# jiaw-z/DKT-Stereo

Measured on AMD Instinct MI355X. Metric: stereo pairs/sec at 736x1248 D=192, 32 iters (RAFT-Stereo test_mode forward), higher is better.
Workload: dtype f32 io/accumulate; convolution products = 3x fp16-split MFMA (22-bit operands); lookup / correlation exact fp32

## Files before the change

dkt_stereo_amd/csrc/resample_c8.hip:

```cpp
#include "dkt_common.h"

__device__ __forceinline__ unsigned rs_pack_h2(_Float16 a, _Float16 b) {
    union { _Float16 h[2]; unsigned u; } v;
    v.h[0] = a;
    v.h[1] = b;
    return v.u;
}

__device__ __forceinline__ void rs_store_c8(char *p, long plane, const float (&v)[8], float scale) {
    unsigned hw[4], lw[4];
#pragma unroll
    for (int d = 0; d < 4; ++d) {
        const float x0 = v[2 * d] * scale, x1 = v[2 * d + 1] * scale;
        const _Float16 a0 = (_Float16)x0, a1 = (_Float16)x1;
        hw[d] = rs_pack_h2(a0, a1);
        lw[d] = rs_pack_h2((_Float16)(x0 - (float)a0), (_Float16)(x1 - (float)a1));
    }
    *(uint4 *)p = make_uint4(hw[0], hw[1], hw[2], hw[3]);
    *(uint4 *)(p + plane) = make_uint4(lw[0], lw[1], lw[2], lw[3]);
}

__device__ __forceinline__ void pool2x_c8_body(const float *__restrict__ x, long x_bs, char *__restrict__ dst, long dst_bs,
                                               int C, int H, int W, int Ho, int Wo, int Wp, long plane, int ch0, float scale,
                                               int bx, int oy, int bz) {
    const int ox = bx * 128 + threadIdx.x;
    const int g = bz % ((C + 7) / 8), b = bz / ((C + 7) / 8);
    if (ox >= Wo) return;
    const float *xb = x + (long)b * x_bs;
    float v[8];
#pragma unroll
    for (int k = 0; k < 8; ++k) {
        const int c = g * 8 + k;
        const float *p = xb + (long)(c < C ? c : C - 1) * H * W;
        float t[9];
#pragma unroll
        for (int dy = 0; dy < 3; ++dy) {
            const int iy = 2 * oy - 1 + dy;
            const bool yok = iy >= 0 && iy < H;
#pragma unroll
            for (int dx = 0; dx < 3; ++dx) {
                const int ix = 2 * ox - 1 + dx;
                const bool ok = yok && ix >= 0 && ix < W;
                const float u = p[(long)(yok ? iy : 0) * W + (ix >= 0 && ix < W ? ix : 0)];
                t[dy * 3 + dx] = ok ? u : 0.0f;
            }
        }
        float s = 0.0f;
#pragma unroll
        for (int i = 0; i < 9; ++i) s = __fadd_rn(s, t[i]);
        v[k] = c < C ? __fdiv_rn(s, 9.0f) : 0.0f;
    }
    rs_store_c8(dst + (long)b * dst_bs + (long)((ch0 >> 3) + g) * 2 * plane + ((long)(oy + 1) * Wp + (ox + 1)) * 16, plane, v, scale);
}

__device__ __forceinline__ void interp_c8_body(const float *__restrict__ x, long x_bs, char *__restrict__ dst, long dst_bs,
                                               int C, int H, int W, int Ho, int Wo, float sy, float sx, int Wp, long plane,
                                               int ch0, float scale, int bx, int oy, int bz) {
    const int ox = bx * 128 + threadIdx.x;
    const int g = bz % ((C + 7) / 8), b = bz / ((C + 7) / 8);
    if (ox >= Wo) return;
    const float fy = __fmul_rn(sy, (float)oy);
    const int y0 = (int)fy;
    const int y1 = y0 + (y0 < H - 1 ? 1 : 0);
    const float ly1 = __fsub_rn(fy, (float)y0), ly0 = __fsub_rn(1.0f, ly1);
    const float fx = __fmul_rn(sx, (float)ox);
    const int x0 = (int)fx;
    const int x1 = x0 + (x0 < W - 1 ? 1 : 0);
    const float lx1 = __fsub_rn(fx, (float)x0), lx0 = __fsub_rn(1.0f, lx1);
    const float *xb = x + (long)b * x_bs;
    float a0[8], a1[8], b0[8], b1[8];
#pragma unroll
    for (int k = 0; k < 8; ++k) {
        const int c = g * 8 + k;
        const float *p = xb + (long)(c < C ? c : C - 1) * H * W;
        a0[k] = p[(long)y0 * W + x0]; a1[k] = p[(long)y0 * W + x1];
        b0[k] = p[(long)y1 * W + x0]; b1[k] = p[(long)y1 * W + x1];
    }
    float v[8];
#pragma unroll
    for (int k = 0; k < 8; ++k) {
        const float top = __fadd_rn(__fmul_rn(lx0, a0[k]), __fmul_rn(lx1, a1[k]));
        const float bot = __fadd_rn(__fmul_rn(lx0, b0[k]), __fmul_rn(lx1, b1[k]));
        v[k] = g * 8 + k < C ? __fadd_rn(__fmul_rn(ly0, top), __fmul_rn(ly1, bot)) : 0.0f;
    }
    rs_store_c8(dst + (long)b * dst_bs + (long)((ch0 >> 3) + g) * 2 * plane + ((long)(oy + 1) * Wp + (ox + 1)) * 16, plane, v, scale);
}

__global__ __launch_bounds__(128) void pool2x_c8_kernel(const float *__restrict__ x, long x_bs, char *__restrict__ dst, long dst_bs,
                                                        int C, int H, int W, int Ho, int Wo, int Wp, long plane, int ch0, float scale) {
    pool2x_c8_body(x, x_bs, dst, dst_bs, C, H, W, Ho, Wo, Wp, plane, ch0, scale, blockIdx.x, blockIdx.y, blockIdx.z);
}

__global__ __launch_bounds__(128) void interp_c8_kernel(const float *__restrict__ x, long x_bs, char *__restrict__ dst, long dst_bs,
                                                        int C, int H, int W, int Ho, int Wo, float sy, float sx, int Wp, long plane,
                                                        int ch0, float scale) {
    interp_c8_body(x, x_bs, dst, dst_bs, C, H, W, Ho, Wo, sy, sx, Wp, plane, ch0, scale, blockIdx.x, blockIdx.y, blockIdx.z);
}

struct RsJob {
    const float *x; long x_bs;
    char *dst; long dst_bs;
    int C, H, W, Ho, Wo, Wp; long plane; int ch0; float scale;
    float sy, sx;
    int kind;
    int nbx, nby;
};
struct RsPair { RsJob j[2]; };

__global__ __launch_bounds__(128) void resample_pair_c8_kernel(RsPair a, int nb0) {
    const bool second = (int)blockIdx.x >= nb0;
    const RsJob &j = a.j[second ? 1 : 0];
    int id = (int)blockIdx.x - (second ? nb0 : 0);
    const int bx = id % j.nbx; id /= j.nbx;
    const int oy = id % j.nby, bz = id / j.nby;
    if (j.kind == 0) pool2x_c8_body(j.x, j.x_bs, j.dst, j.dst_bs, j.C, j.H, j.W, j.Ho, j.Wo, j.Wp, j.plane, j.ch0, j.scale, bx, oy, bz);
    else interp_c8_body(j.x, j.x_bs, j.dst, j.dst_bs, j.C, j.H, j.W, j.Ho, j.Wo, j.sy, j.sx, j.Wp, j.plane, j.ch0, j.scale, bx, oy, bz);
}

static int rs_fill(RsJob &j, const dkt_resample_c8_job *d, long &blocks) {
    if (!d || !d->x || !d->dst) return DKT_E_NULL;
    if (d->B <= 0 || d->C <= 0 || d->H <= 0 || d->W <= 0 || (d->ch0 & 7) || !(d->scale > 0.0f)) return DKT_E_SHAPE;
    if (d->kind != 0 && d->kind != 1) return DKT_E_UNSUPPORTED;
    j.x = d->x; j.x_bs = d->x_bstride; j.dst = (char *)d->dst; j.dst_bs = d->dst_bstride_bytes;
    j.C = d->C; j.H = d->H; j.W = d->W; j.ch0 = d->ch0; j.scale = d->scale; j.kind = d->kind;
    if (d->kind == 0) {
        j.Ho = (d->H - 1) / 2 + 1; j.Wo = (d->W - 1) / 2 + 1;
        j.sy = j.sx = 0.0f;
    } else {
        if (d->Ho <= 0 || d->Wo <= 0) return DKT_E_SHAPE;
        j.Ho = d->Ho; j.Wo = d->Wo;
        j.sy = j.Ho > 1 ? (float)(d->H - 1) / (float)(j.Ho - 1) : 0.0f;
        j.sx = j.Wo > 1 ? (float)(d->W - 1) / (float)(j.Wo - 1) : 0.0f;
    }
    int Hp, Wp;
    dkt_act_c8_dims(j.Ho, j.Wo, &Hp, &Wp);
    j.Wp = Wp; j.plane = (long)Hp * Wp * 16;
    j.nbx = (j.Wo + 127) / 128; j.nby = j.Ho;
    blocks = (long)j.nbx * j.nby * d->B * ((d->C + 7) / 8);
    return DKT_OK;
}

extern "C" int dkt_resample_pair_c8(const dkt_resample_c8_job *job0, const dkt_resample_c8_job *job1, int device, void *stream) {
    RsPair a;
    long n0 = 0, n1 = 0;
    int rc = rs_fill(a.j[0], job0, n0);
    if (rc != DKT_OK) return rc;
    rc = rs_fill(a.j[1], job1, n1);
    if (rc != DKT_OK) return rc;
    if (n0 + n1 > 0x7fffffffL) return DKT_E_SHAPE;
    DKT_ENTER(device);
    hipLaunchKernelGGL(resample_pair_c8_kernel, dim3((unsigned)(n0 + n1)), dim3(128), 0, (hipStream_t)stream, a, (int)n0);
    return dkt_launch_status();
}

extern "C" int dkt_pool2x_c8(const float *x, long x_bstride, void *dst, long dst_bstride_bytes, int B, int C, int H, int W,
                             int ch0, float scale, int device, void *stream) {
    if (!x || !dst) return DKT_E_NULL;
    if (B <= 0 || C <= 0 || H <= 0 || W <= 0 || (ch0 & 7) || !(scale > 0.0f)) return DKT_E_SHAPE;
    const int Ho = (H - 1) / 2 + 1, Wo = (W - 1) / 2 + 1;
    int Hp, Wp;
    dkt_act_c8_dims(Ho, Wo, &Hp, &Wp);
    const long gz = (long)B * ((C + 7) / 8);
    if (gz > 65535 || Ho > 65535) return DKT_E_SHAPE;
    DKT_ENTER(device);
    hipLaunchKernelGGL(pool2x_c8_kernel, dim3((unsigned)((Wo + 127) / 128), (unsigned)Ho, (unsigned)gz), dim3(128), 0, (hipStream_t)stream,
                       x, x_bstride, (char *)dst, dst_bstride_bytes, C, H, W, Ho, Wo, Wp, (long)Hp * Wp * 16, ch0, scale);
    return dkt_launch_status();
}

extern "C" int dkt_interp_c8(const float *x, long x_bstride, void *dst, long dst_bstride_bytes, int B, int C, int H, int W,
                             int Ho, int Wo, int ch0, float scale, int device, void *stream) {
    if (!x || !dst) return DKT_E_NULL;
    if (B <= 0 || C <= 0 || H <= 0 || W <= 0 || Ho <= 0 || Wo <= 0 || (ch0 & 7) || !(scale > 0.0f)) return DKT_E_SHAPE;
    int Hp, Wp;
    dkt_act_c8_dims(Ho, Wo, &Hp, &Wp);
    const long gz = (long)B * ((C + 7) / 8);
    if (gz > 65535 || Ho > 65535) return DKT_E_SHAPE;
    const float sy = Ho > 1 ? (float)(H - 1) / (float)(Ho - 1) : 0.0f;
    const float sx = Wo > 1 ? (float)(W - 1) / (float)(Wo - 1) : 0.0f;
    DKT_ENTER(device);
    hipLaunchKernelGGL(interp_c8_kernel, dim3((unsigned)((Wo + 127) / 128), (unsigned)Ho, (unsigned)gz), dim3(128), 0, (hipStream_t)stream,
                       x, x_bstride, (char *)dst, dst_bstride_bytes, C, H, W, Ho, Wo, sy, sx, Wp, (long)Hp * Wp * 16, ch0, scale);
    return dkt_launch_status();
}
```

Before: 31.57.

## Stage resample input tiles in LDS with strip-based tiling for pool and interp

```diff
diff --git a/dkt_stereo_amd/csrc/resample_c8.hip b/dkt_stereo_amd/csrc/resample_c8.hip
--- a/dkt_stereo_amd/csrc/resample_c8.hip
+++ b/dkt_stereo_amd/csrc/resample_c8.hip
@@ -20,82 +20,10 @@
     *(uint4 *)(p + plane) = make_uint4(lw[0], lw[1], lw[2], lw[3]);
 }
 
-__device__ __forceinline__ void pool2x_c8_body(const float *__restrict__ x, long x_bs, char *__restrict__ dst, long dst_bs,
-                                               int C, int H, int W, int Ho, int Wo, int Wp, long plane, int ch0, float scale,
-                                               int bx, int oy, int bz) {
-    const int ox = bx * 128 + threadIdx.x;
-    const int g = bz % ((C + 7) / 8), b = bz / ((C + 7) / 8);
-    if (ox >= Wo) return;
-    const float *xb = x + (long)b * x_bs;
-    float v[8];
-#pragma unroll
-    for (int k = 0; k < 8; ++k) {
-        const int c = g * 8 + k;
-        const float *p = xb + (long)(c < C ? c : C - 1) * H * W;
-        float t[9];
-#pragma unroll
-        for (int dy = 0; dy < 3; ++dy) {
-            const int iy = 2 * oy - 1 + dy;
-            const bool yok = iy >= 0 && iy < H;
-#pragma unroll
-            for (int dx = 0; dx < 3; ++dx) {
-                const int ix = 2 * ox - 1 + dx;
-                const bool ok = yok && ix >= 0 && ix < W;
-                const float u = p[(long)(yok ? iy : 0) * W + (ix >= 0 && ix < W ? ix : 0)];
-                t[dy * 3 + dx] = ok ? u : 0.0f;
-            }
-        }
-        float s = 0.0f;
-#pragma unroll
-        for (int i = 0; i < 9; ++i) s = __fadd_rn(s, t[i]);
-        v[k] = c < C ? __fdiv_rn(s, 9.0f) : 0.0f;
-    }
-    rs_store_c8(dst + (long)b * dst_bs + (long)((ch0 >> 3) + g) * 2 * plane + ((long)(oy + 1) * Wp + (ox + 1)) * 16, plane, v, scale);
-}
-
-__device__ __forceinline__ void interp_c8_body(const float *__restrict__ x, long x_bs, char *__restrict__ dst, long dst_bs,
-                                               int C, int H, int W, int Ho, int Wo, float sy, float sx, int Wp, long plane,
-                                               int ch0, float scale, int bx, int oy, int bz) {
-    const int ox = bx * 128 + threadIdx.x;
-    const int g = bz % ((C + 7) / 8), b = bz / ((C + 7) / 8);
-    if (ox >= Wo) return;
-    const float fy = __fmul_rn(sy, (float)oy);
-    const int y0 = (int)fy;
-    const int y1 = y0 + (y0 < H - 1 ? 1 : 0);
-    const float ly1 = __fsub_rn(fy, (float)y0), ly0 = __fsub_rn(1.0f, ly1);
-    const float fx = __fmul_rn(sx, (float)ox);
-    const int x0 = (int)fx;
-    const int x1 = x0 + (x0 < W - 1 ? 1 : 0);
-    const float lx1 = __fsub_rn(fx, (float)x0), lx0 = __fsub_rn(1.0f, lx1);
-    const float *xb = x + (long)b * x_bs;
-    float a0[8], a1[8], b0[8], b1[8];
-#pragma unroll
-    for (int k = 0; k < 8; ++k) {
-        const int c = g * 8 + k;
-        const float *p = xb + (long)(c < C ? c : C - 1) * H * W;
-        a0[k] = p[(long)y0 * W + x0]; a1[k] = p[(long)y0 * W + x1];
-        b0[k] = p[(long)y1 * W + x0]; b1[k] = p[(long)y1 * W + x1];
-    }
-    float v[8];
-#pragma unroll
-    for (int k = 0; k < 8; ++k) {
-        const float top = __fadd_rn(__fmul_rn(lx0, a0[k]), __fmul_rn(lx1, a1[k]));
-        const float bot = __fadd_rn(__fmul_rn(lx0, b0[k]), __fmul_rn(lx1, b1[k]));
-        v[k] = g * 8 + k < C ? __fadd_rn(__fmul_rn(ly0, top), __fmul_rn(ly1, bot)) : 0.0f;
-    }
-    rs_store_c8(dst + (long)b * dst_bs + (long)((ch0 >> 3) + g) * 2 * plane + ((long)(oy + 1) * Wp + (ox + 1)) * 16, plane, v, scale);
-}
-
-__global__ __launch_bounds__(128) void pool2x_c8_kernel(const float *__restrict__ x, long x_bs, char *__restrict__ dst, long dst_bs,
-                                                        int C, int H, int W, int Ho, int Wo, int Wp, long plane, int ch0, float scale) {
-    pool2x_c8_body(x, x_bs, dst, dst_bs, C, H, W, Ho, Wo, Wp, plane, ch0, scale, blockIdx.x, blockIdx.y, blockIdx.z);
-}
-
-__global__ __launch_bounds__(128) void interp_c8_kernel(const float *__restrict__ x, long x_bs, char *__restrict__ dst, long dst_bs,
-                                                        int C, int H, int W, int Ho, int Wo, float sy, float sx, int Wp, long plane,
-                                                        int ch0, float scale) {
-    interp_c8_body(x, x_bs, dst, dst_bs, C, H, W, Ho, Wo, sy, sx, Wp, plane, ch0, scale, blockIdx.x, blockIdx.y, blockIdx.z);
-}
+#define RS_THREADS 256
+#define RS_LDS_FLOATS 6144
+#define RS_MAX_ROWS 8
+#define RS_MAX_ITEMS 768
 
 struct RsJob {
     const float *x; long x_bs;
@@ -104,17 +32,141 @@
     float sy, sx;
     int kind;
     int nbx, nby;
+    int R, XS, pitch;
 };
 struct RsPair { RsJob j[2]; };
 
-__global__ __launch_bounds__(128) void resample_pair_c8_kernel(RsPair a, int nb0) {
+#define RS_BATCH 6
+__device__ __forceinline__ void rs_stage(float *lds, const float *__restrict__ xb, int C, int H, int W, int g, int y_lo, int ns,
+                                         int cb, int pitch) {
+    const int Q = pitch >> 2, n = ns * 8 * Q;
+    for (int i0 = threadIdx.x; i0 < n; i0 += RS_BATCH * RS_THREADS) {
+        float4 v[RS_BATCH];
+        int at[RS_BATCH];
+#pragma unroll
+        for (int u = 0; u < RS_BATCH; ++u) {
+            const int i = i0 + u * RS_THREADS;
+            const int rk = i / Q, q = i - rk * Q;
+            const int c = g * 8 + (rk & 7), iy = y_lo + (rk >> 3), ix = cb + 4 * q;
+            at[u] = i < n ? rk * pitch + 4 * q : -1;
+            v[u] = make_float4(0.0f, 0.0f, 0.0f, 0.0f);
+            if (i < n && c < C && iy >= 0 && iy < H) {
+                const float *row = xb + ((long)c * H + iy) * W;
+                if (ix >= 0 && ix + 3 < W && (((uintptr_t)(row + ix)) & 15) == 0) {
+                    v[u] = *(const float4 *)(row + ix);
+                } else {
+                    if (ix >= 0 && ix < W) v[u].x = row[ix];
+                    if (ix + 1 >= 0 && ix + 1 < W) v[u].y = row[ix + 1];
+                    if (ix + 2 >= 0 && ix + 2 < W) v[u].z = row[ix + 2];
+                    if (ix + 3 >= 0 && ix + 3 < W) v[u].w = row[ix + 3];
+                }
+            }
+        }
+#pragma unroll
+        for (int u = 0; u < RS_BATCH; ++u)
+            if (at[u] >= 0) *(float4 *)(lds + at[u]) = v[u];
+    }
+}
+
+__device__ __forceinline__ void pool2x_c8_strip(float *lds, const RsJob &j, int seg, int strip, int bz) {
+    const int G = (j.C + 7) / 8, g = bz % G, b = bz / G;
+    const int oy0 = strip * j.R, nr = min(j.R, j.Ho - oy0);
+    const int ox0 = seg * j.XS, nx = min(j.XS, j.Wo - ox0);
+    const int pitch = j.pitch;
+    rs_stage(lds, j.x + (long)b * j.x_bs, j.C, j.H, j.W, g, 2 * oy0 - 1, 2 * nr + 1, 2 * ox0 - 4, pitch);
+    __syncthreads();
+    char *db = j.dst + (long)b * j.dst_bs + (long)((j.ch0 >> 3) + g) * 2 * j.plane;
+    for (int item = threadIdx.x; item < nr * nx; item += RS_THREADS) {
+        const int r = item / nx, lx = item - r * nx;
+        const float *tap = lds + (long)(2 * r) * 8 * pitch + 2 * lx + 3;
+        float v[8];
+#pragma unroll
+        for (int k = 0; k < 8; ++k) {
+            float t[9];
+#pragma unroll
+            for (int dy = 0; dy < 3; ++dy) {
+                const float *q = tap + (dy * 8 + k) * pitch;
+                const float2 m = *(const float2 *)(q + 1);
+                t[dy * 3] = q[0]; t[dy * 3 + 1] = m.x; t[dy * 3 + 2] = m.y;
+            }
+            float s = 0.0f;
+#pragma unroll
+            for (int i = 0; i < 9; ++i) s = __fadd_rn(s, t[i]);
+            v[k] = g * 8 + k < j.C ? __fdiv_rn(s, 9.0f) : 0.0f;
+        }
+        rs_store_c8(db + ((long)(oy0 + r + 1) * j.Wp + (ox0 + lx + 1)) * 16, j.plane, v, j.scale);
+    }
+}
+
+__device__ __forceinline__ void interp_c8_strip(float *lds, const RsJob &j, int seg, int strip, int bz) {
+    const int G = (j.C + 7) / 8, g = bz % G, b = bz / G;
+    const int H = j.H, W = j.W;
+    const int oy0 = strip * j.R, nr = min(j.R, j.Ho - oy0);
+    const int ox0 = seg * j.XS, nx = min(j.XS, j.Wo - ox0);
+    const int pitch = j.pitch;
+    const int ylo = (int)__fmul_rn(j.sy, (float)oy0);
+    const int ylast = (int)__fmul_rn(j.sy, (float)(oy0 + nr - 1));
+    const int ns = min(ylast + (ylast < H - 1 ? 1 : 0) - ylo + 1, RS_LDS_FLOATS / (8 * pitch));
+    const int cb = (int)__fmul_rn(j.sx, (float)ox0) & ~3;
+    rs_stage(lds, j.x + (long)b * j.x_bs, j.C, H, W, g, ylo, ns, cb, pitch);
+    __syncthreads();
+    char *db = j.dst + (long)b * j.dst_bs + (long)((j.ch0 >> 3) + g) * 2 * j.plane;
+    for (int item = threadIdx.x; item < nr * nx; item += RS_THREADS) {
+        const int r = item / nx, lx = item - r * nx;
+        const int oy = oy0 + r, ox = ox0 + lx;
+        const float fy = __fmul_rn(j.sy, (float)oy);
+        const int y0 = (int)fy;
+        const int y1 = y0 + (y0 < H - 1 ? 1 : 0);
+        const float ly1 = __fsub_rn(fy, (float)y0), ly0 = __fsub_rn(1.0f, ly1);
+        const float fx = __fmul_rn(j.sx, (float)ox);
+        const int x0 = (int)fx;
+        const int x1 = x0 + (x0 < W - 1 ? 1 : 0);
+        const float lx1 = __fsub_rn(fx, (float)x0), lx0 = __fsub_rn(1.0f, lx1);
+        const float *r0 = lds + (long)(y0 - ylo) * 8 * pitch - cb, *r1 = lds + (long)(y1 - ylo) * 8 * pitch - cb;
+        float v[8];
+#pragma unroll
+        for (int k = 0; k < 8; ++k) {
+            const float top = __fadd_rn(__fmul_rn(lx0, r0[k * pitch + x0]), __fmul_rn(lx1, r0[k * pitch + x1]));
+            const float bot = __fadd_rn(__fmul_rn(lx0, r1[k * pitch + x0]), __fmul_rn(lx1, r1[k * pitch + x1]));
+            v[k] = g * 8 + k < j.C ? __fadd_rn(__fmul_rn(ly0, top), __fmul_rn(ly1, bot)) : 0.0f;
+        }
+        rs_store_c8(db + ((long)(oy + 1) * j.Wp + (ox + 1)) * 16, j.plane, v, j.scale);
+    }
+}
+
+__device__ __forceinline__ void rs_run(float *lds, const RsJob &j, int id) {
+    const int seg = id % j.nbx; id /= j.nbx;
+    const int strip = id % j.nby, bz = id / j.nby;
+    if (j.kind == 0) pool2x_c8_strip(lds, j, seg, strip, bz);
+    else interp_c8_strip(lds, j, seg, strip, bz);
+}
+
+__global__ __launch_bounds__(RS_THREADS) void resample_c8_kernel(RsJob j) {
+    __shared__ __attribute__((aligned(16))) float lds[RS_LDS_FLOATS];
+    rs_run(lds, j, (int)blockIdx.x);
+}
+
+__global__ __launch_bounds__(RS_THREADS) void resample_pair_c8_kernel(RsPair a, int nb0) {
+    __shared__ __attribute__((aligned(16))) float lds[RS_LDS_FLOATS];
     const bool second = (int)blockIdx.x >= nb0;
-    const RsJob &j = a.j[second ? 1 : 0];
-    int id = (int)blockIdx.x - (second ? nb0 : 0);
-    const int bx = id % j.nbx; id /= j.nbx;
-    const int oy = id % j.nby, bz = id / j.nby;
-    if (j.kind == 0) pool2x_c8_body(j.x, j.x_bs, j.dst, j.dst_bs, j.C, j.H, j.W, j.Ho, j.Wo, j.Wp, j.plane, j.ch0, j.scale, bx, oy, bz);
-    else interp_c8_body(j.x, j.x_bs, j.dst, j.dst_bs, j.C, j.H, j.W, j.Ho, j.Wo, j.sy, j.sx, j.Wp, j.plane, j.ch0, j.scale, bx, oy, bz);
+    rs_run(lds, a.j[second ? 1 : 0], (int)blockIdx.x - (second ? nb0 : 0));
+}
+
+static void rs_plan(RsJob &j) {
+    auto rows = [&](int R) { return j.kind == 0 ? 2 * R + 1 : (int)((R - 1) * (double)j.sy + 0.01) + 3; };
+    auto pitch = [&](int XS) { return j.kind == 0 ? 2 * XS + 4 : ((int)((XS - 1) * (double)j.sx + 0.01) + 6 + 3) & ~3; };
+    for (int min_r = 2; min_r >= 1; --min_r)
+        for (int nseg = 1; nseg <= j.Wo; ++nseg) {
+            int XS = (j.Wo + nseg - 1) / nseg;
+            if (j.kind == 0) XS = (XS + 1) & ~1;
+            const int P = pitch(XS);
+            int R = j.Ho < RS_MAX_ROWS ? j.Ho : RS_MAX_ROWS;
+            while (R > 1 && ((long)rows(R) * 8 * P > RS_LDS_FLOATS || (R > 2 && R * XS > RS_MAX_ITEMS))) --R;
+            if ((long)rows(R) * 8 * P > RS_LDS_FLOATS || (R < min_r && R < j.Ho)) continue;
+            j.R = R; j.XS = XS; j.pitch = P;
+            j.nbx = (j.Wo + XS - 1) / XS; j.nby = (j.Ho + R - 1) / R;
+            return;
+        }
 }
 
 static int rs_fill(RsJob &j, const dkt_resample_c8_job *d, long &blocks) {
@@ -135,7 +187,7 @@
     int Hp, Wp;
     dkt_act_c8_dims(j.Ho, j.Wo, &Hp, &Wp);
     j.Wp = Wp; j.plane = (long)Hp * Wp * 16;
-    j.nbx = (j.Wo + 127) / 128; j.nby = j.Ho;
+    rs_plan(j);
     blocks = (long)j.nbx * j.nby * d->B * ((d->C + 7) / 8);
     return DKT_OK;
 }
@@ -149,37 +201,29 @@
     if (rc != DKT_OK) return rc;
     if (n0 + n1 > 0x7fffffffL) return DKT_E_SHAPE;
     DKT_ENTER(device);
-    hipLaunchKernelGGL(resample_pair_c8_kernel, dim3((unsigned)(n0 + n1)), dim3(128), 0, (hipStream_t)stream, a, (int)n0);
+    hipLaunchKernelGGL(resample_pair_c8_kernel, dim3((unsigned)(n0 + n1)), dim3(RS_THREADS), 0, (hipStream_t)stream, a, (int)n0);
+    return dkt_launch_status();
+}
+
+static int rs_single(const dkt_resample_c8_job &d, int device, void *stream) {
+    RsJob j;
+    long n = 0;
+    const int rc = rs_fill(j, &d, n);
+    if (rc != DKT_OK) return rc;
+    if ((long)d.B * ((d.C + 7) / 8) > 65535 || j.Ho > 65535 || n > 0x7fffffffL) return DKT_E_SHAPE;
+    DKT_ENTER(device);
+    hipLaunchKernelGGL(resample_c8_kernel, dim3((unsigned)n), dim3(RS_THREADS), 0, (hipStream_t)stream, j);
     return dkt_launch_status();
 }
 
 extern "C" int dkt_pool2x_c8(const float *x, long x_bstride, void *dst, long dst_bstride_bytes, int B, int C, int H, int W,
                              int ch0, float scale, int device, void *stream) {
-    if (!x || !dst) return DKT_E_NULL;
-    if (B <= 0 || C <= 0 || H <= 0 || W <= 0 || (ch0 & 7) || !(scale > 0.0f)) return DKT_E_SHAPE;
-    const int Ho = (H - 1) / 2 + 1, Wo = (W - 1) / 2 + 1;
-    int Hp, Wp;
-    dkt_act_c8_dims(Ho, Wo, &Hp, &Wp);
-    const long gz = (long)B * ((C + 7) / 8);
-    if (gz > 65535 || Ho > 65535) return DKT_E_SHAPE;
-    DKT_ENTER(device);
-    hipLaunchKernelGGL(pool2x_c8_kernel, dim3((unsigned)((Wo + 127) / 128), (unsigned)Ho, (unsigned)gz), dim3(128), 0, (hipStream_t)stream,
-                       x, x_bstride, (char *)dst, dst_bstride_bytes, C, H, W, Ho, Wo, Wp, (long)Hp * Wp * 16, ch0, scale);
-    return dkt_launch_status();
+    dkt_resample_c8_job d = {x, x_bstride, dst, dst_bstride_bytes, B, C, H, W, 0, 0, ch0, 0, scale};
+    return rs_single(d, device, stream);
 }
 
 extern "C" int dkt_interp_c8(const float *x, long x_bstride, void *dst, long dst_bstride_bytes, int B, int C, int H, int W,
                              int Ho, int Wo, int ch0, float scale, int device, void *stream) {
-    if (!x || !dst) return DKT_E_NULL;
-    if (B <= 0 || C <= 0 || H <= 0 || W <= 0 || Ho <= 0 || Wo <= 0 || (ch0 & 7) || !(scale > 0.0f)) return DKT_E_SHAPE;
-    int Hp, Wp;
-    dkt_act_c8_dims(Ho, Wo, &Hp, &Wp);
-    const long gz = (long)B * ((C + 7) / 8);
-    if (gz > 65535 || Ho > 65535) return DKT_E_SHAPE;
-    const float sy = Ho > 1 ? (float)(H - 1) / (float)(Ho - 1) : 0.0f;
-    const float sx = Wo > 1 ? (float)(W - 1) / (float)(Wo - 1) : 0.0f;
-    DKT_ENTER(device);
-    hipLaunchKernelGGL(interp_c8_kernel, dim3((unsigned)((Wo + 127) / 128), (unsigned)Ho, (unsigned)gz), dim3(128), 0, (hipStream_t)stream,
-                       x, x_bstride, (char *)dst, dst_bstride_bytes, C, H, W, Ho, Wo, sy, sx, Wp, (long)Hp * Wp * 16, ch0, scale);
-    return dkt_launch_status();
-}
+    dkt_resample_c8_job d = {x, x_bstride, dst, dst_bstride_bytes, B, C, H, W, Ho, Wo, ch0, 1, scale};
+    return rs_single(d, device, stream);
+}
```

Result: no change. 31.60 (median of 3 runs) (+0.1%).
